# qzed/raft-meets-dicl

Hardware: AMD Instinct MI355X
Metric: frame-pairs/s @436x1024 RAFT 12 iters (1-8 GPU); corr MFMA% + lookup HBM% (higher is better)
Workload: dtype bf16; 1 GPU; RAFT all-pairs correlation + 4-level pyramid + 12 radius-4 lookups (BASELINE configs[1]); the whole network is the 'model_level' key; image=436x1024 padded 440x1024, feature_map=55x128, channels=256, batch_per_gpu=8, global_batch=8, precision=bf16, pyramid_storage=fp16, parallelism=batch-shard x1

## Files before the change

include/rmd.h:

```cpp
#ifndef RMD_H
#define RMD_H

#include <stddef.h>

#ifdef __cplusplus
extern "C" {
#endif

#define RMD_OK 0
#define RMD_ERR_ARG (-1)
#define RMD_ERR_SHAPE (-2)
#define RMD_ERR_LAUNCH (-3)

#define RMD_F32 0
#define RMD_F16 1
#define RMD_BF16 2
#define RMD_BF16X3 3
#define RMD_S24 4

#define RMD_MAX_LEVELS 4

#define RMD_LAYOUT_ROWS 0
#define RMD_LAYOUT_TILES 1

typedef struct rmd_pyramid_desc {
    int batch, height, width;
    int levels;
    int storage;
    int level_h[RMD_MAX_LEVELS], level_w[RMD_MAX_LEVELS];
    int tile_h[RMD_MAX_LEVELS], tile_w[RMD_MAX_LEVELS];
    int tiles_y[RMD_MAX_LEVELS], tiles_x[RMD_MAX_LEVELS];
    long long level_offset[RMD_MAX_LEVELS];
    long long total_elements;
    int layout;
    int query_slots;
} rmd_pyramid_desc;

int rmd_pyramid_describe(int batch, int height, int width, int levels, int storage,
                         rmd_pyramid_desc* desc);

int rmd_pyramid_describe_layout(int batch, int height, int width, int levels, int storage, int layout,
                                rmd_pyramid_desc* desc);

int rmd_pyramid_describe_for(int batch, int height, int width, int levels, int storage, int channels,
                             int compute, rmd_pyramid_desc* desc);

size_t rmd_corr_pyramid_workspace_bytes(const rmd_pyramid_desc* desc, int channels, int compute);

int rmd_corr_pyramid(const float* fmap1, const float* fmap2, int channels, float scale,
                     const rmd_pyramid_desc* desc, int compute, void* pyramid, void* workspace,
                     void* stream);

const char* rmd_corr_gemm_kernel(const rmd_pyramid_desc* desc, int channels, int compute);

int rmd_corr_prepare(const float* fmap1, const float* fmap2, int channels, float scale,
                     const rmd_pyramid_desc* desc, int compute, void* workspace, void* stream);
int rmd_corr_pyramid_prepared(int channels, float scale, const rmd_pyramid_desc* desc, int compute,
                              void* pyramid, void* workspace, void* stream);

int rmd_corr_lookup(const void* pyramid, const rmd_pyramid_desc* desc, const float* coords,
                    int radius, unsigned zero_level_mask, float* out, void* stream);

size_t rmd_corr_otf_workspace_bytes(int batch, int channels, int height, int width, int levels, int compute);
int rmd_corr_otf_prepare(const float* fmap1, const float* fmap2, int batch, int channels, int height, int width,
                         int levels, float scale, int compute, void* workspace, void* stream);
int rmd_corr_otf_lookup(const void* workspace, int batch, int channels, int height, int width, int levels,
                        int compute, const float* coords, int radius, unsigned zero_level_mask, float* out,
                        void* stream);

size_t rmd_corr_otf_record_bytes(int batch, int height, int width, int levels, int radius);
int rmd_corr_otf_record(const float* grad_out, const float* coords, int batch, int height, int width, int levels,
                        int radius, unsigned zero_level_mask, void* record, void* stream);
size_t rmd_corr_otf_backward_workspace_bytes(int batch, int channels, int height, int width, int levels, int compute);
int rmd_corr_otf_backward(const float* fmap1, const float* fmap2, const void* otf_workspace, int batch, int channels,
                          int height, int width, int levels, float scale, int compute, int radius, int nrecords,
                          const void* const* records, float* grad_fmap1, float* grad_fmap2, void* workspace,
                          void* stream);


long long rmd_corr_grad_targets(int height, int width, int levels);

int rmd_corr_lookup_backward(const float* grad_out, const rmd_pyramid_desc* desc, const float* coords,
                             int radius, unsigned zero_level_mask, float* grad_levels, void* stream);

int rmd_corr_grad_build(const float* const* grad_outs, const float* const* coords,
                        const unsigned* zero_level_masks, int nlookups, const rmd_pyramid_desc* desc, int radius,
                        int accumulate, float* grad_levels, void* stream);

int rmd_corr_grad_build_ex(const float* const* grad_outs, const float* const* coords,
                           const unsigned* zero_level_masks, int nlookups, const rmd_pyramid_desc* desc, int radius,
                           int accumulate, int bf16_out, void* grad_levels, void* stream);

int rmd_corr_pool_targets(const float* fmap2, int batch, int channels, int height, int width, int levels,
                          float scale, float* pooled, void* stream);

int rmd_corr_unpool_targets(const float* grad_pooled, int batch, int channels, int height, int width, int levels,
                            float scale, float* grad_fmap2, void* stream);

size_t rmd_corr_grad_gemm_workspace_bytes(int batch, int m, int k, int nc);
int rmd_corr_grad_gemm(const float* a, long long lda, const float* bm, long long ldb, int batch, int m, int k, int nc,
                       int layout, int compute, float* out, void* workspace, void* stream);

int rmd_corr_grad_gemm_bf16g(const float* a, long long lda, const void* bm, long long ldb, int batch, int m, int k,
                             int nc, int layout, float* out, void* workspace, void* stream);


int rmd_dicl_stack(const float* fmap1, const float* fmap2, const float* coords, int batch, int channels,
                   int height, int width, int level_height, int level_width, int radius, int level,
                   int norm_height, int norm_width, int extra_delta, float* out, void* stream);

int rmd_dicl_stack_backward(const float* grad_stack, const float* coords, int batch, int channels,
// ... 201 lines not shown
```

raft-meets-dicl_amd/csrc/corr_pyramid.h:

```cpp
#pragma once

#include "mfma_bf16.h"

namespace rmd {


constexpr int kKC = 64;
inline int padded_channels(int C) { return (C + kKC - 1) / kKC * kKC; }

__device__ __forceinline__ unsigned pack_half2(float a, float b) {
    const __half2 h = __floats2half2_rn(a, b);
    return *reinterpret_cast<const unsigned*>(&h);
}

__device__ __forceinline__ void swap32(unsigned& x, unsigned& y) {
    auto r = __builtin_amdgcn_permlane32_swap(x, y, false, false);
    x = r[0];
    y = r[1];
}

#define RMD_ACC(acc, row, cg, k) (acc[2 * ((row) >> 2) + (cg)][((row) & 3) * 4 + (k)])


namespace x3 {

bool eligible(const rmd_pyramid_desc& d, int channels);
size_t workspace_bytes(const rmd_pyramid_desc& d);
int prepare(const float* fmap1, const float* fmap2, int channels, float scale, const rmd_pyramid_desc& d,
            void* workspace, hipStream_t st);
int pyramid(const rmd_pyramid_desc& d, void* pyramid, void* workspace, hipStream_t st);

}

namespace w8 {

bool eligible(const rmd_pyramid_desc& d, int channels);
int prepare(const float* fmap1, const float* fmap2, int channels, float scale, const rmd_pyramid_desc& d,
            void* workspace, hipStream_t st);
int pyramid(const rmd_pyramid_desc& d, void* pyramid, void* workspace, hipStream_t st);

}

namespace stationary {

bool eligible(const rmd_pyramid_desc& d, int channels);
int pyramid(const rmd_pyramid_desc& d, void* pyramid, void* workspace, hipStream_t st);

}

namespace tiled {

int prepare(const float* fmap1, const float* fmap2, int channels, float scale, const rmd_pyramid_desc& d, int compute,
            void* workspace, hipStream_t st);
int pyramid(int channels, float scale, const rmd_pyramid_desc& d, int compute, void* pyramid, void* workspace,
            hipStream_t st);

}

}
```

raft-meets-dicl_amd/csrc/corr_pyramid.hip:

```cpp

#include "corr_pyramid.h"

namespace rmd {
namespace {

enum class Path { W8, STATIONARY, TILED, X3 };

Path gemm_path(const rmd_pyramid_desc& d, int C, int compute) {
    if (compute == RMD_BF16X3) return x3::eligible(d, C) ? Path::X3 : Path::TILED;
    if (compute == RMD_BF16) {
        if (w8::eligible(d, C)) return Path::W8;
        if (stationary::eligible(d, C)) return Path::STATIONARY;
    }
    return Path::TILED;
}

int path_layout(Path p) { return p == Path::W8 ? RMD_LAYOUT_TILES : RMD_LAYOUT_ROWS; }

int tiled_compute(int compute) { return compute == RMD_BF16X3 ? RMD_F32 : compute; }

int check_args(const rmd_pyramid_desc* d, int channels, int compute) {
    RMD_REQUIRE(d, RMD_ERR_ARG, "rmd_corr_pyramid: null desc");
    RMD_REQUIRE(channels > 0, RMD_ERR_SHAPE, "rmd_corr_pyramid: channels must be > 0");
    RMD_REQUIRE(d->levels >= 1 && d->levels <= RMD_MAX_LEVELS, RMD_ERR_SHAPE, "rmd_corr_pyramid: bad levels");
// ... 26 lines not shown
}

extern "C" size_t rmd_corr_pyramid_workspace_bytes(const rmd_pyramid_desc* d, int channels, int compute) {
    if (!d || channels <= 0) return 0;
    if (compute == RMD_BF16X3) {
        if (rmd::x3::eligible(*d, channels)) return rmd::x3::workspace_bytes(*d);
        compute = RMD_F32;
    }
    const size_t Cp = (size_t)rmd::padded_channels(channels);
    const size_t es = compute == RMD_F32 ? 4 : 2;
    const size_t N = (size_t)d->height * d->width;
    const size_t S = d->query_slots > 0 && (size_t)d->query_slots > N ? (size_t)d->query_slots : N;
    const size_t Npad = (S + 31) / 32 * 32;
    return (size_t)d->batch * (N + Npad) * Cp * es + 32 * 1024;
}

extern "C" const char* rmd_corr_gemm_kernel(const rmd_pyramid_desc* d, int channels, int compute) {
    if (!d || channels <= 0) return "invalid";
    switch (rmd::gemm_path(*d, channels, compute)) {
        case rmd::Path::W8: return "w8";
        case rmd::Path::STATIONARY: return "stationary";
        case rmd::Path::X3: return "x3";
        default: return "tiled";
    }
}

extern "C" int rmd_corr_prepare(const float* fmap1, const float* fmap2, int channels, float scale,
                                const rmd_pyramid_desc* d, int compute, void* workspace, void* stream) {
    RMD_REQUIRE(fmap1 && fmap2 && workspace, RMD_ERR_ARG, "rmd_corr_prepare: null pointer");
    int rc = rmd::check_args(d, channels, compute);
    if (rc) return rc;
    hipStream_t st = rmd::as_stream(stream);
    switch (rmd::gemm_path(*d, channels, compute)) {
        case rmd::Path::X3: return rmd::x3::prepare(fmap1, fmap2, channels, scale, *d, workspace, st);
        case rmd::Path::W8: return rmd::w8::prepare(fmap1, fmap2, channels, scale, *d, workspace, st);
        default: return rmd::tiled::prepare(fmap1, fmap2, channels, scale, *d, rmd::tiled_compute(compute), workspace, st);
    }
}

extern "C" int rmd_corr_pyramid_prepared(int channels, float scale, const rmd_pyramid_desc* d, int compute,
                                         void* pyramid, void* workspace, void* stream) {
    RMD_REQUIRE(pyramid && workspace, RMD_ERR_ARG, "rmd_corr_pyramid_prepared: null pointer");
    int rc = rmd::check_args(d, channels, compute);
    if (rc) return rc;
    hipStream_t st = rmd::as_stream(stream);
    switch (rmd::gemm_path(*d, channels, compute)) {
        case rmd::Path::X3: return rmd::x3::pyramid(*d, pyramid, workspace, st);
        case rmd::Path::W8: return rmd::w8::pyramid(*d, pyramid, workspace, st);
        case rmd::Path::STATIONARY: return rmd::stationary::pyramid(*d, pyramid, workspace, st);
        default: return rmd::tiled::pyramid(channels, scale, *d, rmd::tiled_compute(compute), pyramid, workspace, st);
    }
}

extern "C" int rmd_corr_pyramid(const float* fmap1, const float* fmap2, int channels, float scale,
                                const rmd_pyramid_desc* d, int compute, void* pyramid, void* workspace, void* stream) {
    int rc = rmd_corr_prepare(fmap1, fmap2, channels, scale, d, compute, workspace, stream);
    if (rc) return rc;
    return rmd_corr_pyramid_prepared(channels, scale, d, compute, pyramid, workspace, stream);
}
```

raft-meets-dicl_amd/csrc/corr_pyramid_w8.hip:

```cpp

#include "corr_pyramid.h"

namespace rmd {
namespace {

constexpr int kPrepPx = 128, kPrepStride = 256 * 2 + 16;

__global__ void __launch_bounds__(512)
prep_pair(const float* __restrict__ f1, const float* __restrict__ f2, __bf16* __restrict__ opA,
          __bf16* __restrict__ opB, int C, int H, int W, int S, int nqt, float scale) {
    extern __shared__ __attribute__((aligned(16))) unsigned char lds[];
    const int b = blockIdx.y, which = blockIdx.z;
    const int N = H * W;
    const float* f = which ? f1 : f2;
    const float s = which ? 1.0f : scale;
    const int t = threadIdx.x;
    const int p0 = blockIdx.x * kPrepPx;
    if (p0 >= (which ? S : N)) return;
#pragma unroll
    for (int it = 0; it < 2; ++it) {
        const int item = it * 512 + t;
        const int q = item & 31, cg = item >> 5;
        int y1, x1;
        if (which) {
            tiles_pixel(p0 + 4 * q, H, W, y1, x1);
        } else {
            y1 = 0;
            x1 = p0 + 4 * q;
        }
        const int lim = which ? W : N;
        const bool full = (which ? y1 < H : true) && x1 + 3 < lim && (lim & 3) == 0;
        const int yc = which ? min(y1, H - 1) : 0;
        const float* src = f + ((size_t)b * C) * N + (size_t)yc * (which ? W : 0);
        float v[8][4];
#pragma unroll
        for (int e = 0; e < 8; ++e) {
            const int c = cg * 8 + e;
            const float* row = src + (size_t)c * N;
            float4 x = make_float4(0.f, 0.f, 0.f, 0.f);
            if (c < C) {
                if (full) {
                    x = *reinterpret_cast<const float4*>(row + x1);
                } else {
                    x.x = row[min(x1 + 0, lim - 1)];
                    x.y = row[min(x1 + 1, lim - 1)];
                    x.z = row[min(x1 + 2, lim - 1)];
                    x.w = row[min(x1 + 3, lim - 1)];
                }
            }
            v[e][0] = x.x * s;
            v[e][1] = x.y * s;
            v[e][2] = x.z * s;
            v[e][3] = x.w * s;
        }
#pragma unroll
        for (int i = 0; i < 4; ++i) {
            bf16x8 o;
#pragma unroll
            for (int e = 0; e < 8; ++e) o[e] = (__bf16)v[e][i];
            *reinterpret_cast<bf16x8*>(lds + (size_t)(4 * q + i) * kPrepStride + cg * 16) = o;
        }
    }
    __syncthreads();
#pragma unroll
    for (int it = 0; it < 8; ++it) {
        const int k = it * 512 + t;
        int px, c0;
        if (which) {
            const int L = k & 63, st = (k >> 6) & 15;
            px = (k >> 10) * 32 + (L & 31);
            c0 = 16 * st + 8 * (L >> 5);
        } else {
            px = k >> 5;
            c0 = (k & 31) * 8;
        }
        const bf16x8 o = *reinterpret_cast<const bf16x8*>(lds + (size_t)px * kPrepStride + c0 * 2);
        if (which) {
            const int qt = blockIdx.x * 4 + (k >> 10);
            if (qt < nqt) *reinterpret_cast<bf16x8*>(opB + (((size_t)b * nqt + qt) * 1024 + (k & 1023)) * 8) = o;
        } else if (p0 + px < N) {
            *reinterpret_cast<bf16x8*>(opA + ((size_t)b * N + p0) * 256 + (size_t)k * 8) = o;
        }
    }
}


constexpr unsigned kBig = 0x40000000u;

constexpr int kStoreAux = 2;

struct Lvl {
    __amdgpu_buffer_rsrc_t rsrc;
    unsigned rs;
    unsigned cs;
    unsigned hd;
    int nq;
};

struct Ctx {
    Lvl l[4];
};

struct LaneOff {
    unsigned o0[2];
    unsigned o1;
    unsigned o2;
    unsigned o3;
};

__device__ __forceinline__ LaneOff lane_offsets(const Ctx& c, int q, int h) {
    LaneOff r;
    const unsigned uq = (unsigned)q;
#pragma unroll
    for (int tc = 0; tc < 2; ++tc)
        r.o0[tc] = 2 * tc + h < c.l[0].nq ? uq * 16u + (unsigned)(2 * tc + h) * c.l[0].cs : kBig;
    r.o1 = h < c.l[1].nq ? uq * 16u + (unsigned)h * c.l[1].cs : kBig;
    r.o2 = c.l[2].nq > 0 ? uq * 8u + (unsigned)h * c.l[2].rs : kBig;
    r.o3 = c.l[3].nq > 0 ? uq * 4u + (unsigned)h * (c.l[3].rs + c.l[3].hd) : kBig;
    return r;
}

struct EpiState {
    float s1[8][2][2];
    float s2[4][2];
};

#define V(row, cg, k) RMD_ACC(acc, row, cg, k)

template <int S>
__device__ __forceinline__ void epi_piece(const f32x16 (&acc)[8], const Ctx& c, const LaneOff& lo, EpiState& st) {
    constexpr int m = S >> 1, tc = S & 1;
    {
        const i32x4 d = {(int)pack_half2(V(2 * m, tc, 0), V(2 * m, tc, 1)),
                         (int)pack_half2(V(2 * m, tc, 2), V(2 * m, tc, 3)),
                         (int)pack_half2(V(2 * m + 1, tc, 0), V(2 * m + 1, tc, 1)),
                         (int)pack_half2(V(2 * m + 1, tc, 2), V(2 * m + 1, tc, 3))};
        __builtin_amdgcn_raw_buffer_store_b128(d, c.l[0].rsrc,
                                               (int)(lo.o0[tc] + (unsigned)m * c.l[0].rs + (m >= 4 ? c.l[0].hd : 0u)),
// ... 40 lines not shown
        swap32(x1, y1);
        const float inv = 1.0f / 64.0f;
        const unsigned v = pack_half2(inv * (__uint_as_float(x0) + __uint_as_float(y0)),
                                      inv * (__uint_as_float(x1) + __uint_as_float(y1)));
        __builtin_amdgcn_raw_buffer_store_b32((int)v, c.l[3].rsrc, (int)lo.o3, 0, kStoreAux);
    }
}
#undef V

constexpr unsigned kPadRow = 528;

__device__ __forceinline__ int pad_row(int y, int x) { return ((x >> 3) << 7) + (y << 3) + (x & 7); }

constexpr int kEpiStores = 24;
constexpr int kRing = 8;

template <int S>
__device__ __forceinline__ void read_a8(bf16x8 (&a)[8], const unsigned char* smem, unsigned b0, unsigned b1) {
#pragma unroll
    for (int ti = 0; ti < 8; ++ti)
        a[ti] = *reinterpret_cast<const bf16x8*>(smem + ((ti & 1) ? b1 : b0) + (unsigned)((ti >> 1) * 32 * kPadRow + 32 * S));
}

template <int S>
__device__ __forceinline__ void ksteps_ring(f32x16 (&acc)[8], bf16x8 (&acur)[8], bf16x8 (&anext)[8],
                                            bf16x8 (&ring)[kRing], const unsigned char* smem, unsigned b0,
                                            unsigned b1, const __bf16* cur, const __bf16* nxt) {
    if constexpr (S < 16) {
        if constexpr (S + 1 < 16) read_a8<S + 1>(anext, smem, b0, b1);
        {
            constexpr int T = S + kRing - 1;
            ring[T % kRing] = *reinterpret_cast<const bf16x8*>((T < 16 ? cur : nxt) + 512 * (T & 15));
        }
        const f32x16 zero = {};
#pragma unroll
        for (int ti = 0; ti < 8; ++ti)
            acc[ti] = __builtin_amdgcn_mfma_f32_32x32x16_bf16(acur[ti], ring[S % kRing], S == 0 ? zero : acc[ti], 0, 0, 0);
        if constexpr (S + 1 < 16) __builtin_amdgcn_sched_group_barrier(0x100, 8, 0);
        __builtin_amdgcn_sched_group_barrier(0x020, 1, 0);
        __builtin_amdgcn_sched_group_barrier(0x008, 8, 0);
        __builtin_amdgcn_sched_barrier(0);
        ksteps_ring<S + 1>(acc, anext, acur, ring, smem, b0, b1, cur, nxt);
    }
}

template <int S>
__device__ __forceinline__ void epilogue(const f32x16 (&acc)[8], const Ctx& c, const LaneOff& lo, EpiState& st) {
    if constexpr (S < 16) {
        epi_piece<S>(acc, c, lo, st);
        epilogue<S + 1>(acc, c, lo, st);
    }
}

struct Bal {
    int pair;
    int nwg;
};

__global__ void __launch_bounds__(512, 1)
corr_pyramid_w8(const __bf16* __restrict__ opA, const __bf16* __restrict__ opB, PyrGeom g, int qsplit,
                __half* __restrict__ pyr, Bal bal) {
    constexpr int Cp = 256, CPR = Cp / 8, WAVES = 8;
    extern __shared__ __attribute__((aligned(16))) unsigned char smem[];

    const int H = g.height, W = g.width, N = H * W;
    const int ncb = (W + 15) >> 4;
    const int nrb = (H + 15) >> 4;
    const int nqt = g.slots >> 5;
    const int nfull = bal.pair ? (nrb - 1) * ncb : nrb * ncb;
    const int nblk = nfull + (bal.pair ? ncb / 2 : 0);
    const int lid = xcd_block(blockIdx.x, bal.nwg);
    const int ib = lid % nblk;
    const int rest = lid / nblk;
    const int split = rest % qsplit;
    const int b = rest / qsplit;
    const bool paired = ib >= nfull;
    const int tb = paired ? (nrb - 1) * ncb + 2 * (ib - nfull) : ib;
    const int rb = tb / ncb, cb = tb - rb * ncb;
    const int ty0 = rb * 16, tx0 = cb * 16;
    const int tid = threadIdx.x, lane = tid & 63;
    const int w = __builtin_amdgcn_readfirstlane(tid >> 6);
    const int j = lane & 31, h = lane >> 5;

    const __bf16* gA = opA + (size_t)b * N * Cp;
    constexpr int kPieces = 256 * CPR / (64 * WAVES);
    uint4 av[kPieces];
#pragma unroll
    for (int i = 0; i < kPieces; ++i) {
        const int id = tid + i * 64 * WAVES;
        const int row = id / CPR, c = id - row * CPR;
        const bool second = paired && (row >> 4) >= 8;
        const int ty = ty0 + (row >> 4) - (second ? 8 : 0), tx = tx0 + (row & 15) + (second ? 16 : 0);
        av[i] = make_uint4(0, 0, 0, 0);
        if (ty < H && tx < W) av[i] = *reinterpret_cast<const uint4*>(gA + (size_t)(ty * W + tx) * Cp + c * 8);
    }
#pragma unroll
    for (int i = 0; i < kPieces; ++i) {
        const int id = tid + i * 64 * WAVES;
        const int row = id / CPR, c = id - row * CPR;
        *reinterpret_cast<uint4*>(smem + (size_t)pad_row(row >> 4, row & 15) * kPadRow + c * 16) = av[i];
    }
    __syncthreads();

    const unsigned pb0 = (unsigned)j * kPadRow + 16u * h, pb1 = pb0 + 128u * kPadRow;

    Ctx c;
    const unsigned S = (unsigned)g.slots;
#pragma unroll
    for (int l = 0; l < 4; ++l) {
        const int crows = l <= 1 ? 8 >> l : 4 >> (l - 2);
        const int cpb = l == 0 ? 4 : (l == 1 ? 2 : 1);
        const int cbytes = l <= 1 ? 16 : (l == 2 ? 8 : 4);
        const int cr0 = rb * crows, cc0 = cb * cpb;
        const bool lv = l < g.levels;
        const int rows = lv ? max(0, min(crows, g.ty[l] - cr0)) : 0;
        const unsigned cs = S * (unsigned)cbytes;
        const unsigned rs = lv ? (unsigned)g.tx[l] * cs : 0u;
        const size_t base = lv ? ((size_t)g.off[l] * 2 + (((size_t)b * g.ty[l] + cr0) * g.tx[l] + cc0) * (size_t)cs) : 0;
        const unsigned char* bp = reinterpret_cast<const unsigned char*>(pyr) + base;
        const unsigned lo32 = __builtin_amdgcn_readfirstlane((unsigned)(uintptr_t)bp);
        const unsigned hi32 = __builtin_amdgcn_readfirstlane((unsigned)((uintptr_t)bp >> 32));
        c.l[l].rsrc = __builtin_amdgcn_make_buffer_rsrc(reinterpret_cast<void*>(((uintptr_t)hi32 << 32) | lo32), (short)0,
                                                        (int)__builtin_amdgcn_readfirstlane((unsigned)rows * rs), 0x00020000);
        c.l[l].rs = __builtin_amdgcn_readfirstlane(rs);
        c.l[l].cs = __builtin_amdgcn_readfirstlane(cs);
        c.l[l].nq = __builtin_amdgcn_readfirstlane(lv ? max(0, min(cpb, g.tx[l] - cc0)) : 0);
        c.l[l].hd = paired ? __builtin_amdgcn_readfirstlane((unsigned)cpb * cs - (unsigned)(crows / 2) * rs) : 0u;
    }

    const __bf16* gB = opB + ((size_t)b * nqt * 1024 + lane) * 8;
    const int stride = WAVES * qsplit;
    const int f0 = split * WAVES;
    int qt = f0 + w;
    const int nmax = f0 < nqt ? (nqt - f0 + stride - 1) / stride : 0;
    const int nw = qt < nqt ? (nqt - qt + stride - 1) / stride : 0;
    const bool late = w >= 4;
    unsigned b0 = pb0, b1 = pb1;
    asm volatile("" : "+v"(b0), "+v"(b1));
    bf16x8 ring[kRing];
    if (nw > 0) {
#pragma unroll
        for (int s = 0; s < kRing - 1; ++s) ring[s] = *reinterpret_cast<const bf16x8*>(gB + (size_t)qt * 8192 + 512 * s);
    }
    vmcnt_pad_n<kEpiStores>(pyr);
    if (late) __builtin_amdgcn_s_barrier();
    for (int k = 0; k < nmax; ++k) {
        f32x16 acc[8];
        const int qn = qt + stride;
        if (k < nw) {
            bf16x8 a0[8], a1[8];
            read_a8<0>(a0, smem, b0, b1);
            ksteps_ring<0>(acc, a0, a1, ring, smem, b0, b1, gB + (size_t)qt * 8192,
                           gB + (size_t)min(qn, nqt - 1) * 8192);
            __builtin_amdgcn_s_barrier();
            const LaneOff lo = lane_offsets(c, qt * 32 + j, h);
            EpiState st;
            epilogue<0>(acc, c, lo, st);
            __builtin_amdgcn_s_barrier();
            qt = qn;
            continue;
        }
        __builtin_amdgcn_s_barrier();
        __builtin_amdgcn_s_barrier();
        qt = qn;
    }
    if (!late) __builtin_amdgcn_s_barrier();
}

long long tiles_slots(int H, int W) {
    return (long long)(H / 2) * ((W + 15) / 16) * 32 + ((H & 1) ? (long long)(W + 31) / 32 * 32 : 0);
}

Bal w8_balance(const rmd_pyramid_desc& d, int qs) {
    const int nrb = (d.height + 15) / 16, ncb = (d.width + 15) / 16;
    const int rows_last = d.height - 16 * (nrb - 1);
    if (qs == 1 && nrb >= 2 && rows_last <= 8 && d.width % 32 == 0) return {1, ((nrb - 1) * ncb + ncb / 2) * d.batch};
    return {0, nrb * ncb * d.batch * qs};
}

}

namespace w8 {

bool eligible(const rmd_pyramid_desc& d, int channels) {
    if (d.storage != RMD_F16 || padded_channels(channels) != 256) return false;
    const double slots = (double)tiles_slots(d.height, d.width);
    const double span0 = 16.0 * ((d.width + 7) / 8 * 8) * slots * 2;
    return span0 < (double)(1u << 30);
}

int prepare(const float* fmap1, const float* fmap2, int channels, float scale, const rmd_pyramid_desc& d,
            void* workspace, hipStream_t st) {
    const int N = d.height * d.width;
    __bf16* opA = reinterpret_cast<__bf16*>(workspace);
    __bf16* opB = opA + (size_t)d.batch * N * 256;
    const int S = d.query_slots;
    const int nqt = S / 32;
    const int lds = kPrepPx * kPrepStride;
    const int nx = ((N > S ? N : S) + kPrepPx - 1) / kPrepPx;
    (void)hipFuncSetAttribute(reinterpret_cast<const void*>(prep_pair), hipFuncAttributeMaxDynamicSharedMemorySize, lds);
    prep_pair<<<dim3(nx, d.batch, 2), 512, lds, st>>>(fmap1, fmap2, opA, opB, channels, d.height, d.width, S, nqt, scale);
    return check_launch("rmd_corr_prepare");
}

int pyramid(const rmd_pyramid_desc& d, void* pyramid, void* workspace, hipStream_t st) {
    const int N = d.height * d.width;
    __bf16* opA = reinterpret_cast<__bf16*>(workspace);
    __bf16* opB = opA + (size_t)d.batch * N * 256;
    const int nblk = ((d.height + 15) / 16) * ((d.width + 15) / 16);
    const int nqt = d.query_slots / 32;
    int qs = 1;
    while (nblk * d.batch * qs < 256 && qs * 32 <= nqt) qs *= 2;
    const int lds = 256 * (int)kPadRow;
    const Bal bal = w8_balance(d, qs);
    (void)hipFuncSetAttribute(reinterpret_cast<const void*>(corr_pyramid_w8), hipFuncAttributeMaxDynamicSharedMemorySize, lds);
    corr_pyramid_w8<<<bal.nwg, 512, lds, st>>>(opA, opB, make_geom(d), qs, reinterpret_cast<__half*>(pyramid), bal);
    return check_launch("rmd_corr_pyramid/gemm-w8");
}

}
}
```

raft-meets-dicl_amd/rmd/_lib.py:

```python

import ctypes
import hashlib
import os

import torch

RMD_OK = 0
RMD_F32, RMD_F16, RMD_BF16, RMD_BF16X3, RMD_S24 = 0, 1, 2, 3, 4
RMD_LAYOUT_ROWS, RMD_LAYOUT_TILES = 0, 1
RMD_NORM_NONE, RMD_NORM_INSTANCE = 0, 1
MAX_LEVELS = 4

_HERE = os.path.dirname(os.path.abspath(__file__))
LIB_PATH = os.environ.get("RMD_LIBRARY", os.path.join(_HERE, "librmd.so"))


class PyramidDesc(ctypes.Structure):

    _fields_ = [
        ("batch", ctypes.c_int), ("height", ctypes.c_int), ("width", ctypes.c_int),
        ("levels", ctypes.c_int), ("storage", ctypes.c_int),
        ("level_h", ctypes.c_int * MAX_LEVELS), ("level_w", ctypes.c_int * MAX_LEVELS),
        ("tile_h", ctypes.c_int * MAX_LEVELS), ("tile_w", ctypes.c_int * MAX_LEVELS),
        ("tiles_y", ctypes.c_int * MAX_LEVELS), ("tiles_x", ctypes.c_int * MAX_LEVELS),
        ("level_offset", ctypes.c_longlong * MAX_LEVELS),
        ("total_elements", ctypes.c_longlong),
        ("layout", ctypes.c_int), ("query_slots", ctypes.c_int),
    ]


LOSS_MAX_PREDICTIONS = 32
RMD_LOSS_L1, RMD_LOSS_L2, RMD_LOSS_ABSMEAN, RMD_LOSS_ROBUST = 1, 2, 3, 4


class LossPrediction(ctypes.Structure):

    _fields_ = [
        ("flow", ctypes.c_void_p), ("mask", ctypes.c_void_p), ("grad", ctypes.c_void_p),
        ("height", ctypes.c_int), ("width", ctypes.c_int), ("weight", ctypes.c_float),
    ]


METRICS_MAX_ESTIMATES, METRICS_MAX_DISTANCES, METRICS_SLOTS = 32, 8, 16


class RmdError(RuntimeError):
    pass


_lib = None

_P = ctypes.c_void_p
_I = ctypes.c_int
_U = ctypes.c_uint
_SIGS = {
    "rmd_pyramid_describe": (_I, [_I, _I, _I, _I, _I, ctypes.POINTER(PyramidDesc)]),
    "rmd_pyramid_describe_layout": (_I, [_I, _I, _I, _I, _I, _I, ctypes.POINTER(PyramidDesc)]),
    "rmd_pyramid_describe_for": (_I, [_I, _I, _I, _I, _I, _I, _I, ctypes.POINTER(PyramidDesc)]),
    "rmd_corr_pyramid_workspace_bytes": (ctypes.c_size_t, [ctypes.POINTER(PyramidDesc), _I, _I]),
    "rmd_corr_pyramid": (_I, [_P, _P, _I, ctypes.c_float, ctypes.POINTER(PyramidDesc), _I, _P, _P, _P]),
    "rmd_corr_lookup": (_I, [_P, ctypes.POINTER(PyramidDesc), _P, _I, _U, _P, _P]),
    "rmd_corr_gemm_kernel": (ctypes.c_char_p, [ctypes.POINTER(PyramidDesc), _I, _I]),
    "rmd_corr_prepare": (_I, [_P, _P, _I, ctypes.c_float, ctypes.POINTER(PyramidDesc), _I, _P, _P]),
    "rmd_corr_pyramid_prepared": (_I, [_I, ctypes.c_float, ctypes.POINTER(PyramidDesc), _I, _P, _P, _P]),
    "rmd_corr_otf_workspace_bytes": (ctypes.c_size_t, [_I] * 6),
    "rmd_corr_otf_prepare": (_I, [_P, _P] + [_I] * 5 + [ctypes.c_float, _I, _P, _P]),
    "rmd_corr_otf_lookup": (_I, [_P] + [_I] * 6 + [_P, _I, _U, _P, _P]),
    "rmd_corr_otf_record_bytes": (ctypes.c_size_t, [_I] * 5),
    "rmd_corr_otf_record": (_I, [_P, _P] + [_I] * 5 + [_U, _P, _P]),
    "rmd_corr_otf_backward_workspace_bytes": (ctypes.c_size_t, [_I] * 6),
    "rmd_corr_otf_backward": (_I, [_P, _P, _P] + [_I] * 5 + [ctypes.c_float, _I, _I, _I, ctypes.POINTER(_P), _P, _P,
                                                               _P, _P]),
    "rmd_corr_grad_targets": (ctypes.c_longlong, [_I, _I, _I]),
    "rmd_corr_lookup_backward": (_I, [_P, ctypes.POINTER(PyramidDesc), _P, _I, _U, _P, _P]),
    "rmd_corr_grad_build": (_I, [ctypes.POINTER(_P), ctypes.POINTER(_P), ctypes.POINTER(_U), _I,
                                 ctypes.POINTER(PyramidDesc), _I, _I, _P, _P]),
    "rmd_corr_grad_build_ex": (_I, [ctypes.POINTER(_P), ctypes.POINTER(_P), ctypes.POINTER(_U), _I,
                                    ctypes.POINTER(PyramidDesc), _I, _I, _I, _P, _P]),
    "rmd_corr_grad_gemm_bf16g": (_I, [_P, ctypes.c_longlong, _P, ctypes.c_longlong, _I, _I, _I, _I, _I, _P, _P, _P]),
    "rmd_corr_pool_targets": (_I, [_P, _I, _I, _I, _I, _I, ctypes.c_float, _P, _P]),
    "rmd_corr_unpool_targets": (_I, [_P, _I, _I, _I, _I, _I, ctypes.c_float, _P, _P]),
    "rmd_corr_grad_gemm_workspace_bytes": (ctypes.c_size_t, [_I, _I, _I, _I]),
    "rmd_corr_grad_gemm": (_I, [_P, ctypes.c_longlong, _P, ctypes.c_longlong, _I, _I, _I, _I, _I, _I, _P, _P, _P]),
    "rmd_dicl_stack": (_I, [_P, _P, _P] + [_I] * 11 + [_P, _P]),
    "rmd_dicl_stack_backward": (_I, [_P, _P] + [_I] * 11 + [_P, _P, _P]),
    "rmd_dicl_stack_kernel": (ctypes.c_char_p, [_I] * 12),
    "rmd_dicl_stack_kernel_list": (ctypes.c_char_p, [_I]),
    "rmd_dicl_stack_int_workspace_bytes": (ctypes.c_size_t, [_I, _I, _I]),
    "rmd_dicl_stack_int": (_I, [_P, _P] + [_I] * 6 + [_P, _P, _P]),
    "rmd_dicl_stack_int_backward": (_I, [_P, _P] + [_I] * 6 + [_P, _P, _P, _P]),
    "rmd_warp_backwards": (_I, [_P, _P, _I, _I, _I, _I, ctypes.c_float, _P, _P, _P]),
    "rmd_warp_backwards_backward": (_I, [_P, _P, _I, _I, _I, _I, ctypes.c_float, _P, _P]),
    "rmd_dicl_stack_int_warped_workspace_bytes": (ctypes.c_size_t, [_I, _I, _I, _I]),
    "rmd_dicl_stack_int_warped": (_I, [_P, _P, _P] + [_I] * 6 + [_P, _P, _P]),
    "rmd_dicl_stack_int_warped_backward": (_I, [_P, _P, _P] + [_I] * 6 + [_P, _P, _P, _P]),
    "rmd_dap": (_I, [_P, _P, _I, _I, _I, _I, _P, _P]),
    "rmd_dap_weight_grad_workspace_bytes": (ctypes.c_size_t, [_I, _I, _I]),
    "rmd_dap_weight_grad": (_I, [_P, _P, _I, _I, _I, _P, _P, _P]),
    "rmd_input_images": (_I, [_P, _I, _I, _I, _I, ctypes.c_float, ctypes.c_float, ctypes.c_float, ctypes.c_float,
                              _I, _I, _I, _I, _I, _P, _P]),
    "rmd_input_flow": (_I, [_P, _P, _I, _I, _I, _I, _I, _I, _I, ctypes.c_float, _P, _P, _P]),
    "rmd_up8": (_I, [_P, _P, _I, _I, _I, ctypes.c_float, _P, _P]),
    "rmd_up8_workspace_bytes": (ctypes.c_size_t, [_I, _I, _I]),
    "rmd_up8_backward": (_I, [_P, _P, _P, _I, _I, _I, ctypes.c_float, _P, _P, _P, _P]),
    "rmd_softargmax": (_I, [_P, _I, _I, _I, _I, _I, ctypes.c_float, _P, _P]),
    "rmd_softargmax_backward": (_I, [_P, _P, _I, _I, _I, _I, _I, ctypes.c_float, _P, _P]),
    "rmd_dicl_flow_head": (_I, [_P, _P, _I, _I, _I, _I, ctypes.c_float, _P, _P]),
    "rmd_dicl_flow_head_backward": (_I, [_P, _P, _I, _I, _I, _I, ctypes.c_float, _P, _P]),
    "rmd_dicl_match_1x1_supported": (_I, [_I] * 5),
    "rmd_dicl_match_1x1_workspace_bytes": (ctypes.c_size_t, [_I] * 5),
    "rmd_dicl_match_1x1": (_I, [_P, _P, _P] + [_I] * 5 + [_P] * 8 + [_I] * 4 + [_P, _P, _P]),
    "rmd_dicl_match_1x1_backward_supported": (_I, [_I] * 5),
    "rmd_dicl_match_1x1_backward_workspace_bytes": (ctypes.c_size_t, [_I] * 8),
    "rmd_dicl_match_1x1_backward": (_I, [_P] * 4 + [_I] * 5 + [_P] * 7 + [_I] * 4 + [_P] * 12),
    "rmd_sepconv_gru_supported": (_I, [_I] * 2),
    "rmd_sepconv_gru_workspace_bytes": (ctypes.c_size_t, [_I] * 5),
    "rmd_sepconv_gru": (_I, [_P] * 6 + [_I] * 6 + [_P]),
# ... 133 lines not shown
```

raft-meets-dicl_amd/rmd/library.py:

```python

import ctypes

import torch

from . import _lib

LIB = torch.library.Library("rmd", "DEF")

_OPS = {
    "corr_pyramid": ("model", "(Tensor fmap1, Tensor fmap2, int levels, int compute, int storage, float scale) "
                              "-> Tensor"),
    "corr_lookup": ("model", "(Tensor pyramid, Tensor coords, int levels, int radius, int level_mask) -> Tensor"),
    "corr_otf_prepare": ("model", "(Tensor fmap1, Tensor fmap2, int levels, int compute, float scale) -> Tensor"),
    "corr_otf_lookup": ("model", "(Tensor workspace, Tensor coords, int channels, int levels, int compute, int radius, "
                                 "int level_mask) -> Tensor"),
    "dicl_stack": ("model", "(Tensor fmap1, Tensor fmap2, Tensor coords, int radius, int level, int norm_h, "
                            "int norm_w, bool extra_delta) -> Tensor"),
    "dicl_stack_backward": ("model", "(Tensor grad, Tensor coords, int channels, int level_h, int level_w, int radius, "
                                     "int level, int norm_h, int norm_w, bool extra_delta) -> (Tensor, Tensor)"),
    "dicl_stack_int": ("model", "(Tensor fmap1, Tensor fmap2, int ru, int rv) -> Tensor"),
    "dicl_stack_int_backward": ("model", "(Tensor grad, Tensor fmap2, int ru, int rv) -> (Tensor, Tensor)"),
    "dicl_stack_int_warped": ("model", "(Tensor fmap1, Tensor fmap2, Tensor flow, int ru, int rv) -> Tensor"),
    "dicl_stack_int_warped_backward": ("model", "(Tensor grad, Tensor fmap2, Tensor flow, int ru, int rv) "
                                                "-> (Tensor, Tensor)"),
# ... 164 lines not shown
    elif pyramid.dim() == 2 and pyramid.shape[1] == TILES_ROW:
        return _lib.RMD_LAYOUT_TILES
    raise ValueError(f"corr_lookup: a pyramid is 1-D (row layout), (n, {TILES_ROW}) (tiles layout) or uint8 "
                     f"(n, {S24_BYTES}) (S24 storage), got {pyramid.dtype} {tuple(pyramid.shape)}")


def pyramid_storage(pyramid):
    if pyramid.dtype not in _STORAGE_CODE:
        raise ValueError(f"corr_lookup: pyramid dtype must be float32, float16 or uint8 (S24), got {pyramid.dtype}")
    return _STORAGE_CODE[pyramid.dtype]


def pyramid_elements(pyramid):
    return pyramid.shape[0] if pyramid.dtype == torch.uint8 else pyramid.numel()


def new_pyramid(like, d):
    if d.storage == _lib.RMD_S24:
        return like.new_empty((d.total_elements, S24_BYTES), dtype=torch.uint8)
    return pyramid_view(like.new_empty((d.total_elements,), dtype=_STORAGE[d.storage]), d.layout)


def pyramid_buffers(f1, levels, compute, storage):
    b, c, h, w = f1.shape
    d = describe_for(b, h, w, levels, storage, c, compute)
    ws = _lib.workspace("corr_pyramid", f1, ctypes.byref(d), c, compute)
    return d, new_pyramid(f1, d), ws


def s24_encode(x):
    u = _f32(x).reshape(-1).view(torch.int32)
    nan = (u & 0x7fffffff) > 0x7f800000
    r = torch.where(nan, u | 0x00400000, u + 0x80)
    return r.view(torch.uint8).view(-1, 4)[:, 1:4].contiguous()


def s24_decode(b):
    w = torch.zeros((b.shape[0], 4), dtype=torch.uint8, device=b.device)
    w[:, 1:4] = b
    return w.view(torch.float32).reshape(-1)



def _check_fmaps(f1, f2):
    if f1.shape != f2.shape or f1.dim() != 4:
        raise ValueError(f"fmap1/fmap2 must be equal (B,C,H,W) shapes, got {tuple(f1.shape)} / {tuple(f2.shape)}")


@_hip("corr_pyramid")
def _corr_pyramid(fmap1, fmap2, levels, compute, storage, scale):
    _check_fmaps(fmap1, fmap2)
    f1, f2 = _f32(fmap1), _f32(fmap2)
    d, data, ws = pyramid_buffers(f1, levels, compute, storage)
    _lib.launch("rmd_corr_pyramid", f1, f1, f2, f1.shape[1], float(scale), ctypes.byref(d), compute, data, ws)
    return data


@_fake("corr_pyramid")
def _(fmap1, fmap2, levels, compute, storage, scale):
    _check_fmaps(fmap1, fmap2)
    b, c, h, w = fmap1.shape
    if fmap1.device.type == "cpu":
        d = describe(b, h, w, levels, _lib.RMD_F32 if storage == _lib.RMD_S24 else storage)
    else:
        d = describe_for(b, h, w, levels, storage, c, compute)
    return new_pyramid(fmap1, d)


def _lookup_out(coords, levels, radius):
    b, _, h, w = coords.shape
    return _like(coords, (b, levels * (2 * radius + 1) ** 2, h, w))


@_hip("corr_lookup")
def _corr_lookup(pyramid, coords, levels, radius, level_mask):
    b, two, h, w = coords.shape
    if pyramid.dtype not in _STORAGE_CODE or not pyramid.is_contiguous():
        raise ValueError(f"corr_lookup: pyramid must be a contiguous float32/float16/uint8 (S24) tensor, got "
                         f"{pyramid.dtype} {tuple(pyramid.shape)}")
    d = describe(b, h, w, levels, pyramid_storage(pyramid), pyramid_layout(pyramid))
    if two != 2 or pyramid_elements(pyramid) != d.total_elements:
        raise ValueError(f"corr_lookup: coords {tuple(coords.shape)} do not match the pyramid ({pyramid.numel()} elements)")
    co = _f32(coords)
    out = _lookup_out(co, levels, radius)
    _lib.launch("rmd_corr_lookup", co, pyramid, ctypes.byref(d), co, radius, level_mask, out)
    return out


@_fake("corr_lookup")
def _(pyramid, coords, levels, radius, level_mask):
    pyramid_layout(pyramid)
    return _lookup_out(coords, levels, radius)


@_hip("corr_otf_prepare")
def _corr_otf_prepare(fmap1, fmap2, levels, compute, scale):
    _check_fmaps(fmap1, fmap2)
    f1, f2 = _f32(fmap1), _f32(fmap2)
    b, c, h, w = f1.shape
    ws = _lib.workspace("corr_otf", f1, b, c, h, w, levels, compute)
    if ws.numel() == 0:
        raise ValueError(f"otf: unsupported sizes {tuple(f1.shape)} with {levels} levels")
    _lib.launch("rmd_corr_otf_prepare", f1, f1, f2, b, c, h, w, levels, float(scale), compute, ws)
    return ws


@_fake("corr_otf_prepare")
# ... 1430 lines not shown
```

raft-meets-dicl_amd/rmd/ops.py:

```python

import ctypes

import torch

from . import _lib, config, library
from ._lib import RMD_BF16, RMD_BF16X3, RMD_F16, RMD_F32, RMD_S24
from .library import _f32

PRECISIONS = {
    "fp32": (RMD_BF16X3, RMD_S24),
    "fp32-f32": (RMD_BF16X3, RMD_F32),
    "fp32-s24": (RMD_BF16X3, RMD_S24),
    "fp32-exact": (RMD_F32, RMD_F32),
    "bf16": (RMD_BF16, RMD_F16),
    "bf16-f32": (RMD_BF16, RMD_F32),
    "fp32-f16": (RMD_F32, RMD_F16),
}


def set_default_precision(name):
    if name not in PRECISIONS:
        raise ValueError(f"unknown precision '{name}', expected one of {sorted(PRECISIONS)}")
    config.configure(precision=name)

# ... 21 lines not shown

class Pyramid:

    def __init__(self, data, desc, channels, scale):
        self.data = data
        self.desc = desc
        self.channels = channels
        self.scale = scale

    @property
    def levels(self):
        return self.desc.levels

    def level_shape(self, i):
        return self.desc.level_h[i], self.desc.level_w[i]

    def unpack(self, i):
        d = self.desc
        b, h, w = d.batch, d.height, d.width
        th, tw, ty, tx = d.tile_h[i], d.tile_w[i], d.tiles_y[i], d.tiles_x[i]
        hl, wl = d.level_h[i], d.level_w[i]
        s = d.query_slots
        off = d.level_offset[i]
        flat = library.s24_decode(self.data) if d.storage == RMD_S24 else self.data.reshape(-1)
        x = flat[off: off + b * ty * tx * s * th * tw].view(b, ty, tx, s, th, tw)
        x = x.permute(0, 3, 1, 4, 2, 5).reshape(b, s, ty * th, tx * tw)[..., :hl, :wl]
        if d.layout == _lib.RMD_LAYOUT_TILES:
            x = x.index_select(1, torch.as_tensor(tiles_slots(h, w), device=x.device))
        return x.float().reshape(b, h, w, 1, hl, wl)


def tiles_slots(h, w):
    y1, x1 = torch.meshgrid(torch.arange(h), torch.arange(w), indexing="ij")
    qx, hp = (w + 15) // 16, h // 2
    s = ((y1 // 2) * qx + x1 // 16) * 32 + ((x1 % 16) // 4) * 8 + (y1 % 2) * 4 + x1 % 4
    s = torch.where(y1 < 2 * hp, s, hp * qx * 32 + x1)
    return s.reshape(-1)


def corr_pyramid(fmap1, fmap2, levels=4, precision=None, events=None, scale=None):
    _same_device(fmap1, fmap2)
    if fmap1.shape != fmap2.shape or fmap1.dim() != 4:
        raise ValueError(f"fmap1/fmap2 must be equal (B,C,H,W) shapes, got {tuple(fmap1.shape)} / {tuple(fmap2.shape)}")
    compute, storage = PRECISIONS[precision or get_default_precision()]
    b, c, h, w = fmap1.shape
    scale = 1.0 / float(c) ** 0.5 if scale is None else float(scale)
    if events is None:
        data = torch.ops.rmd.corr_pyramid(fmap1, fmap2, levels, compute, storage, scale)
        d = library.describe(b, h, w, levels, library.pyramid_storage(data), library.pyramid_layout(data))
        return Pyramid(data, d, c, scale)
    _require_gpu(fmap1, fmap2)
    f1, f2 = _f32(fmap1), _f32(fmap2)
    d, data, ws = library.pyramid_buffers(f1, levels, compute, storage)
    with torch.cuda.device(f1.device):
        _lib.launch("rmd_corr_prepare", f1, f1, f2, c, scale, ctypes.byref(d), compute, ws)
        e0, e1 = torch.cuda.Event(enable_timing=True), torch.cuda.Event(enable_timing=True)
        e0.record()
        _lib.launch("rmd_corr_pyramid_prepared", f1, c, scale, ctypes.byref(d), compute, data, ws)
        e1.record()
        events.append((e0, e1))
    return Pyramid(data, d, c, scale)


def corr_lookup(pyr, coords, radius, mask_costs=()):
    _same_device(pyr.data, coords)
    d = pyr.desc
    if tuple(coords.shape) != (d.batch, 2, d.height, d.width):
        raise ValueError(f"coords must be (B,2,H,W)=({d.batch},2,{d.height},{d.width}), got {tuple(coords.shape)}")
    return torch.ops.rmd.corr_lookup(pyr.data, coords, d.levels, radius, _mask_bits(mask_costs, d.levels))



class OtfState:

    def __init__(self, ws, b, c, h, w, levels, compute):
        self.ws, self.b, self.c, self.h, self.w, self.levels, self.compute = ws, b, c, h, w, levels, compute


def otf_prepare(fmap1, fmap2, levels, precision=None, scale=1.0):
    _same_device(fmap1, fmap2)
    if fmap1.shape != fmap2.shape or fmap1.dim() != 4:
        raise ValueError(f"fmap1/fmap2 must be equal (B,C,H,W) shapes, got {tuple(fmap1.shape)} / {tuple(fmap2.shape)}")
    compute = PRECISIONS[precision or get_default_precision()][0]
    b, c, h, w = fmap1.shape
    ws = torch.ops.rmd.corr_otf_prepare(fmap1, fmap2, levels, compute, float(scale))
    return OtfState(ws, b, c, h, w, levels, compute)


def otf_lookup(st, coords, radius, mask_costs=()):
    _same_device(st.ws, coords)
    if tuple(coords.shape) != (st.b, 2, st.h, st.w):
        raise ValueError(f"coords must be (B,2,H,W)=({st.b},2,{st.h},{st.w}), got {tuple(coords.shape)}")
    return torch.ops.rmd.corr_otf_lookup(st.ws, coords, st.c, st.levels, st.compute, radius,
                                         _mask_bits(mask_costs, st.levels))



class _OtfState:
    def __init__(self, otf, f1, f2, scale):
        self.otf = otf
        self.f1 = f1
        self.f2 = f2
        self.scale = scale
        self.records = []
        self.radius = None


class _OtfPrepareFn(torch.autograd.Function):

    @staticmethod
    def forward(ctx, fmap1, fmap2, state):
# ... 545 lines not shown
```

Before: 15010 frame-pairs/s.

## Fuse fmap2 fp32-to-bf16 staging into the w8 correlation GEMM

```diff
diff --git a/include/rmd.h b/include/rmd.h
--- a/include/rmd.h
+++ b/include/rmd.h
@@ -57,6 +57,15 @@
                      const rmd_pyramid_desc* desc, int compute, void* workspace, void* stream);
 int rmd_corr_pyramid_prepared(int channels, float scale, const rmd_pyramid_desc* desc, int compute,
                               void* pyramid, void* workspace, void* stream);
+
+int rmd_corr_pyramid_fused(const float* fmap1, const float* fmap2, int channels, float scale,
+                           const rmd_pyramid_desc* desc, int compute, void* pyramid, void* workspace,
+                           void* stream);
+
+int rmd_corr_prepare_queries(const float* fmap1, int channels, const rmd_pyramid_desc* desc, int compute,
+                             void* workspace, void* stream);
+int rmd_corr_pyramid_staged(const float* fmap2, int channels, float scale, const rmd_pyramid_desc* desc,
+                            int compute, void* pyramid, void* workspace, void* stream);
 
 int rmd_corr_lookup(const void* pyramid, const rmd_pyramid_desc* desc, const float* coords,
                     int radius, unsigned zero_level_mask, float* out, void* stream);
diff --git a/raft-meets-dicl_amd/csrc/corr_pyramid.h b/raft-meets-dicl_amd/csrc/corr_pyramid.h
--- a/raft-meets-dicl_amd/csrc/corr_pyramid.h
+++ b/raft-meets-dicl_amd/csrc/corr_pyramid.h
@@ -38,6 +38,9 @@
 int prepare(const float* fmap1, const float* fmap2, int channels, float scale, const rmd_pyramid_desc& d,
             void* workspace, hipStream_t st);
 int pyramid(const rmd_pyramid_desc& d, void* pyramid, void* workspace, hipStream_t st);
+int prepare_queries(const float* fmap1, int channels, const rmd_pyramid_desc& d, void* workspace, hipStream_t st);
+int pyramid_staged(const float* fmap2, int channels, float scale, const rmd_pyramid_desc& d, void* pyramid,
+                   void* workspace, hipStream_t st);
 
 }
 
diff --git a/raft-meets-dicl_amd/csrc/corr_pyramid.hip b/raft-meets-dicl_amd/csrc/corr_pyramid.hip
--- a/raft-meets-dicl_amd/csrc/corr_pyramid.hip
+++ b/raft-meets-dicl_amd/csrc/corr_pyramid.hip
@@ -102,6 +102,39 @@
     }
 }
 
+extern "C" int rmd_corr_prepare_queries(const float* fmap1, int channels, const rmd_pyramid_desc* d, int compute,
+                                        void* workspace, void* stream) {
+    RMD_REQUIRE(fmap1 && workspace, RMD_ERR_ARG, "rmd_corr_prepare_queries: null pointer");
+    int rc = rmd::check_args(d, channels, compute);
+    if (rc) return rc;
+    RMD_REQUIRE(rmd::gemm_path(*d, channels, compute) == rmd::Path::W8, RMD_ERR_ARG,
+                "rmd_corr_prepare_queries: the w8 GEMM only (see rmd_corr_gemm_kernel)");
+    return rmd::w8::prepare_queries(fmap1, channels, *d, workspace, rmd::as_stream(stream));
+}
+
+extern "C" int rmd_corr_pyramid_staged(const float* fmap2, int channels, float scale, const rmd_pyramid_desc* d,
+                                       int compute, void* pyramid, void* workspace, void* stream) {
+    RMD_REQUIRE(fmap2 && pyramid && workspace, RMD_ERR_ARG, "rmd_corr_pyramid_staged: null pointer");
+    int rc = rmd::check_args(d, channels, compute);
+    if (rc) return rc;
+    RMD_REQUIRE(rmd::gemm_path(*d, channels, compute) == rmd::Path::W8, RMD_ERR_ARG,
+                "rmd_corr_pyramid_staged: the w8 GEMM only (see rmd_corr_gemm_kernel)");
+    return rmd::w8::pyramid_staged(fmap2, channels, scale, *d, pyramid, workspace, rmd::as_stream(stream));
+}
+
+extern "C" int rmd_corr_pyramid_fused(const float* fmap1, const float* fmap2, int channels, float scale,
+                                      const rmd_pyramid_desc* d, int compute, void* pyramid, void* workspace,
+                                      void* stream) {
+    RMD_REQUIRE(fmap1 && fmap2 && pyramid && workspace, RMD_ERR_ARG, "rmd_corr_pyramid_fused: null pointer");
+    int rc = rmd::check_args(d, channels, compute);
+    if (rc) return rc;
+    if (rmd::gemm_path(*d, channels, compute) != rmd::Path::W8)
+        return rmd_corr_pyramid(fmap1, fmap2, channels, scale, d, compute, pyramid, workspace, stream);
+    rc = rmd::w8::prepare_queries(fmap1, channels, *d, workspace, rmd::as_stream(stream));
+    if (rc) return rc;
+    return rmd::w8::pyramid_staged(fmap2, channels, scale, *d, pyramid, workspace, rmd::as_stream(stream));
+}
+
 extern "C" int rmd_corr_pyramid(const float* fmap1, const float* fmap2, int channels, float scale,
                                 const rmd_pyramid_desc* d, int compute, void* pyramid, void* workspace, void* stream) {
     int rc = rmd_corr_prepare(fmap1, fmap2, channels, scale, d, compute, workspace, stream);
diff --git a/raft-meets-dicl_amd/csrc/corr_pyramid_w8.hip b/raft-meets-dicl_amd/csrc/corr_pyramid_w8.hip
--- a/raft-meets-dicl_amd/csrc/corr_pyramid_w8.hip
+++ b/raft-meets-dicl_amd/csrc/corr_pyramid_w8.hip
@@ -6,11 +6,10 @@
 
 constexpr int kPrepPx = 128, kPrepStride = 256 * 2 + 16;
 
-__global__ void __launch_bounds__(512)
-prep_pair(const float* __restrict__ f1, const float* __restrict__ f2, __bf16* __restrict__ opA,
-          __bf16* __restrict__ opB, int C, int H, int W, int S, int nqt, float scale) {
+__device__ __forceinline__ void prep_tile(const int which, const float* f1, const float* f2, __bf16* opA, __bf16* opB,
+                                          int C, int H, int W, int S, int nqt, float scale) {
     extern __shared__ __attribute__((aligned(16))) unsigned char lds[];
-    const int b = blockIdx.y, which = blockIdx.z;
+    const int b = blockIdx.y;
     const int N = H * W;
     const float* f = which ? f1 : f2;
     const float s = which ? 1.0f : scale;
@@ -84,6 +83,17 @@
     }
 }
 
+__global__ void __launch_bounds__(512)
+prep_pair(const float* __restrict__ f1, const float* __restrict__ f2, __bf16* __restrict__ opA,
+          __bf16* __restrict__ opB, int C, int H, int W, int S, int nqt, float scale) {
+    prep_tile(blockIdx.z, f1, f2, opA, opB, C, H, W, S, nqt, scale);
+}
+
+__global__ void __launch_bounds__(512)
+prep_queries(const float* __restrict__ f1, __bf16* __restrict__ opB, int C, int H, int W, int S, int nqt) {
+    prep_tile(1, f1, nullptr, nullptr, opB, C, H, W, S, nqt, 1.0f);
+}
+
 
 constexpr unsigned kBig = 0x40000000u;
 
@@ -230,14 +240,70 @@
     }
 }
 
+struct StageItem {
+    int xq, cg, y;
+    int ty, tx;
+};
+
+__device__ __forceinline__ StageItem stage_item(int id, int ty0, int tx0, bool paired) {
+    StageItem t;
+    t.xq = id & 3, t.cg = (id >> 2) & 31, t.y = id >> 7;
+    const bool second = paired && t.y >= 8;
+    t.ty = ty0 + t.y - (second ? 8 : 0), t.tx = tx0 + 4 * t.xq + (second ? 16 : 0);
+    return t;
+}
+
+__device__ __forceinline__ void stage_write_px(unsigned char* smem, const StageItem& t, int i, const float (&p)[8], int C,
+                                               int H, int W, float scale) {
+    bf16x8 o;
+#pragma unroll
+    for (int e = 0; e < 8; ++e) o[e] = (__bf16)(t.ty < H && t.tx + i < W ? (t.cg * 8 + e < C ? p[e] : 0.0f) * scale : 0.0f);
+    *reinterpret_cast<bf16x8*>(smem + (size_t)pad_row(t.y, 4 * t.xq + i) * kPadRow + t.cg * 16) = o;
+}
+
+__device__ __forceinline__ void stage_a_f32(unsigned char* smem, const float* __restrict__ f2, int C, int H, int W,
+                                            float scale, int ty0, int tx0, bool paired, int tid) {
+    constexpr int kItems = 4;
+    const int N = H * W;
+    if ((W & 3) == 0 && (reinterpret_cast<uintptr_t>(f2) & 15) == 0 && N < (1 << 22)) {
+#pragma unroll 1
+        for (int it = 0; it < kItems; ++it) {
+            const StageItem t = stage_item(it * 512 + tid, ty0, tx0, paired);
+            const unsigned pix = (unsigned)(min(t.ty, H - 1) * W + min(t.tx, W - 4));
+            float4 x[8];
+#pragma unroll
+            for (int e = 0; e < 8; ++e) {
+                const unsigned c = (unsigned)min(t.cg * 8 + e, C - 1);
+                x[e] = *reinterpret_cast<const float4*>(reinterpret_cast<const unsigned char*>(f2) +
+                                                        (size_t)((c * (unsigned)N + pix) * 4u));
+            }
+            stage_write_px(smem, t, 0, {x[0].x, x[1].x, x[2].x, x[3].x, x[4].x, x[5].x, x[6].x, x[7].x}, C, H, W, scale);
+            stage_write_px(smem, t, 1, {x[0].y, x[1].y, x[2].y, x[3].y, x[4].y, x[5].y, x[6].y, x[7].y}, C, H, W, scale);
+            stage_write_px(smem, t, 2, {x[0].z, x[1].z, x[2].z, x[3].z, x[4].z, x[5].z, x[6].z, x[7].z}, C, H, W, scale);
+            stage_write_px(smem, t, 3, {x[0].w, x[1].w, x[2].w, x[3].w, x[4].w, x[5].w, x[6].w, x[7].w}, C, H, W, scale);
+        }
+        return;
+    }
+#pragma unroll 1
+    for (int k = 0; k < 4 * kItems; ++k) {
+        const StageItem t = stage_item((k >> 2) * 512 + tid, ty0, tx0, paired);
+        const int i = k & 3;
+        const float* px = f2 + (size_t)min(t.ty, H - 1) * W + min(t.tx + i, W - 1);
+        float p[8];
+#pragma unroll
+        for (int e = 0; e < 8; ++e) p[e] = px[(size_t)min(t.cg * 8 + e, C - 1) * N];
+        stage_write_px(smem, t, i, p, C, H, W, scale);
+    }
+}
+
 struct Bal {
     int pair;
     int nwg;
 };
 
-__global__ void __launch_bounds__(512, 1)
-corr_pyramid_w8(const __bf16* __restrict__ opA, const __bf16* __restrict__ opB, PyrGeom g, int qsplit,
-                __half* __restrict__ pyr, Bal bal) {
+template <bool kF32>
+__device__ __forceinline__ void w8_body(const void* srcA, int C, float scale, const __bf16* opB, const PyrGeom& g,
+                                        int qsplit, __half* pyr, const Bal& bal) {
     constexpr int Cp = 256, CPR = Cp / 8, WAVES = 8;
     extern __shared__ __attribute__((aligned(16))) unsigned char smem[];
 
@@ -260,23 +326,27 @@
     const int w = __builtin_amdgcn_readfirstlane(tid >> 6);
     const int j = lane & 31, h = lane >> 5;
 
-    const __bf16* gA = opA + (size_t)b * N * Cp;
-    constexpr int kPieces = 256 * CPR / (64 * WAVES);
-    uint4 av[kPieces];
-#pragma unroll
-    for (int i = 0; i < kPieces; ++i) {
-        const int id = tid + i * 64 * WAVES;
-        const int row = id / CPR, c = id - row * CPR;
-        const bool second = paired && (row >> 4) >= 8;
-        const int ty = ty0 + (row >> 4) - (second ? 8 : 0), tx = tx0 + (row & 15) + (second ? 16 : 0);
-        av[i] = make_uint4(0, 0, 0, 0);
-        if (ty < H && tx < W) av[i] = *reinterpret_cast<const uint4*>(gA + (size_t)(ty * W + tx) * Cp + c * 8);
-    }
-#pragma unroll
-    for (int i = 0; i < kPieces; ++i) {
-        const int id = tid + i * 64 * WAVES;
-        const int row = id / CPR, c = id - row * CPR;
-        *reinterpret_cast<uint4*>(smem + (size_t)pad_row(row >> 4, row & 15) * kPadRow + c * 16) = av[i];
+    if constexpr (kF32) {
+        stage_a_f32(smem, static_cast<const float*>(srcA) + (size_t)b * C * N, C, H, W, scale, ty0, tx0, paired, tid);
+    } else {
+        const __bf16* gA = static_cast<const __bf16*>(srcA) + (size_t)b * N * Cp;
+        constexpr int kPieces = 256 * CPR / (64 * WAVES);
+        uint4 av[kPieces];
+#pragma unroll
+        for (int i = 0; i < kPieces; ++i) {
+            const int id = tid + i * 64 * WAVES;
+            const int row = id / CPR, c = id - row * CPR;
+            const bool second = paired && (row >> 4) >= 8;
+            const int ty = ty0 + (row >> 4) - (second ? 8 : 0), tx = tx0 + (row & 15) + (second ? 16 : 0);
+            av[i] = make_uint4(0, 0, 0, 0);
+            if (ty < H && tx < W) av[i] = *reinterpret_cast<const uint4*>(gA + (size_t)(ty * W + tx) * Cp + c * 8);
+        }
+#pragma unroll
+        for (int i = 0; i < kPieces; ++i) {
+            const int id = tid + i * 64 * WAVES;
+            const int row = id / CPR, c = id - row * CPR;
+            *reinterpret_cast<uint4*>(smem + (size_t)pad_row(row >> 4, row & 15) * kPadRow + c * 16) = av[i];
+        }
     }
     __syncthreads();
 
@@ -345,6 +415,18 @@
     if (!late) __builtin_amdgcn_s_barrier();
 }
 
+__global__ void __launch_bounds__(512, 1)
+corr_pyramid_w8(const __bf16* __restrict__ opA, const __bf16* __restrict__ opB, PyrGeom g, int qsplit,
+                __half* __restrict__ pyr, Bal bal) {
+    w8_body<false>(opA, 0, 0.0f, opB, g, qsplit, pyr, bal);
+}
+
+__global__ void __launch_bounds__(512, 1)
+corr_pyramid_w8_f32(const float* __restrict__ f2, const __bf16* __restrict__ opB, PyrGeom g, int qsplit,
+                    __half* __restrict__ pyr, Bal bal, int C, float scale) {
+    w8_body<true>(f2, C, scale, opB, g, qsplit, pyr, bal);
+}
+
 long long tiles_slots(int H, int W) {
     return (long long)(H / 2) * ((W + 15) / 16) * 32 + ((H & 1) ? (long long)(W + 31) / 32 * 32 : 0);
 }
@@ -381,7 +463,21 @@
     return check_launch("rmd_corr_prepare");
 }
 
-int pyramid(const rmd_pyramid_desc& d, void* pyramid, void* workspace, hipStream_t st) {
+int prepare_queries(const float* fmap1, int channels, const rmd_pyramid_desc& d, void* workspace, hipStream_t st) {
+    const int N = d.height * d.width;
+    __bf16* opB = reinterpret_cast<__bf16*>(workspace) + (size_t)d.batch * N * 256;
+    const int S = d.query_slots;
+    const int lds = kPrepPx * kPrepStride;
+    (void)hipFuncSetAttribute(reinterpret_cast<const void*>(prep_queries), hipFuncAttributeMaxDynamicSharedMemorySize, lds);
+    prep_queries<<<dim3((S + kPrepPx - 1) / kPrepPx, d.batch), 512, lds, st>>>(fmap1, opB, channels, d.height, d.width, S,
+                                                                                S / 32);
+    return check_launch("rmd_corr_prepare_queries");
+}
+
+namespace {
+
+int launch_gemm(const float* fmap2, int channels, float scale, const rmd_pyramid_desc& d, void* pyramid, void* workspace,
+                hipStream_t st) {
     const int N = d.height * d.width;
     __bf16* opA = reinterpret_cast<__bf16*>(workspace);
     __bf16* opB = opA + (size_t)d.batch * N * 256;
@@ -391,10 +487,28 @@
     while (nblk * d.batch * qs < 256 && qs * 32 <= nqt) qs *= 2;
     const int lds = 256 * (int)kPadRow;
     const Bal bal = w8_balance(d, qs);
+    if (fmap2) {
+        (void)hipFuncSetAttribute(reinterpret_cast<const void*>(corr_pyramid_w8_f32),
+                                  hipFuncAttributeMaxDynamicSharedMemorySize, lds);
+        corr_pyramid_w8_f32<<<bal.nwg, 512, lds, st>>>(fmap2, opB, make_geom(d), qs, reinterpret_cast<__half*>(pyramid), bal,
+                                                       channels, scale);
+        return check_launch("rmd_corr_pyramid/gemm-w8-f32");
+    }
     (void)hipFuncSetAttribute(reinterpret_cast<const void*>(corr_pyramid_w8), hipFuncAttributeMaxDynamicSharedMemorySize, lds);
     corr_pyramid_w8<<<bal.nwg, 512, lds, st>>>(opA, opB, make_geom(d), qs, reinterpret_cast<__half*>(pyramid), bal);
     return check_launch("rmd_corr_pyramid/gemm-w8");
 }
 
 }
-}
+
+int pyramid(const rmd_pyramid_desc& d, void* pyramid, void* workspace, hipStream_t st) {
+    return launch_gemm(nullptr, 0, 0.0f, d, pyramid, workspace, st);
+}
+
+int pyramid_staged(const float* fmap2, int channels, float scale, const rmd_pyramid_desc& d, void* pyramid,
+                   void* workspace, hipStream_t st) {
+    return launch_gemm(fmap2, channels, scale, d, pyramid, workspace, st);
+}
+
+}
+}
diff --git a/raft-meets-dicl_amd/rmd/_lib.py b/raft-meets-dicl_amd/rmd/_lib.py
--- a/raft-meets-dicl_amd/rmd/_lib.py
+++ b/raft-meets-dicl_amd/rmd/_lib.py
@@ -63,6 +63,9 @@
     "rmd_corr_gemm_kernel": (ctypes.c_char_p, [ctypes.POINTER(PyramidDesc), _I, _I]),
     "rmd_corr_prepare": (_I, [_P, _P, _I, ctypes.c_float, ctypes.POINTER(PyramidDesc), _I, _P, _P]),
     "rmd_corr_pyramid_prepared": (_I, [_I, ctypes.c_float, ctypes.POINTER(PyramidDesc), _I, _P, _P, _P]),
+    "rmd_corr_pyramid_fused": (_I, [_P, _P, _I, ctypes.c_float, ctypes.POINTER(PyramidDesc), _I, _P, _P, _P]),
+    "rmd_corr_prepare_queries": (_I, [_P, _I, ctypes.POINTER(PyramidDesc), _I, _P, _P]),
+    "rmd_corr_pyramid_staged": (_I, [_P, _I, ctypes.c_float, ctypes.POINTER(PyramidDesc), _I, _P, _P, _P]),
     "rmd_corr_otf_workspace_bytes": (ctypes.c_size_t, [_I] * 6),
     "rmd_corr_otf_prepare": (_I, [_P, _P] + [_I] * 5 + [ctypes.c_float, _I, _P, _P]),
     "rmd_corr_otf_lookup": (_I, [_P] + [_I] * 6 + [_P, _I, _U, _P, _P]),
diff --git a/raft-meets-dicl_amd/rmd/library.py b/raft-meets-dicl_amd/rmd/library.py
--- a/raft-meets-dicl_amd/rmd/library.py
+++ b/raft-meets-dicl_amd/rmd/library.py
@@ -240,7 +240,7 @@
     _check_fmaps(fmap1, fmap2)
     f1, f2 = _f32(fmap1), _f32(fmap2)
     d, data, ws = pyramid_buffers(f1, levels, compute, storage)
-    _lib.launch("rmd_corr_pyramid", f1, f1, f2, f1.shape[1], float(scale), ctypes.byref(d), compute, data, ws)
+    _lib.launch("rmd_corr_pyramid_fused", f1, f1, f2, f1.shape[1], float(scale), ctypes.byref(d), compute, data, ws)
     return data
 
 
diff --git a/raft-meets-dicl_amd/rmd/ops.py b/raft-meets-dicl_amd/rmd/ops.py
--- a/raft-meets-dicl_amd/rmd/ops.py
+++ b/raft-meets-dicl_amd/rmd/ops.py
@@ -97,11 +97,18 @@
     _require_gpu(fmap1, fmap2)
     f1, f2 = _f32(fmap1), _f32(fmap2)
     d, data, ws = library.pyramid_buffers(f1, levels, compute, storage)
+    staged = _lib.lib().rmd_corr_gemm_kernel(ctypes.byref(d), c, compute) == b"w8"
     with torch.cuda.device(f1.device):
-        _lib.launch("rmd_corr_prepare", f1, f1, f2, c, scale, ctypes.byref(d), compute, ws)
+        if staged:
+            _lib.launch("rmd_corr_prepare_queries", f1, f1, c, ctypes.byref(d), compute, ws)
+        else:
+            _lib.launch("rmd_corr_prepare", f1, f1, f2, c, scale, ctypes.byref(d), compute, ws)
         e0, e1 = torch.cuda.Event(enable_timing=True), torch.cuda.Event(enable_timing=True)
         e0.record()
-        _lib.launch("rmd_corr_pyramid_prepared", f1, c, scale, ctypes.byref(d), compute, data, ws)
+        if staged:
+            _lib.launch("rmd_corr_pyramid_staged", f1, f2, c, scale, ctypes.byref(d), compute, data, ws)
+        else:
+            _lib.launch("rmd_corr_pyramid_prepared", f1, c, scale, ctypes.byref(d), compute, data, ws)
         e1.record()
         events.append((e0, e1))
     return Pyramid(data, d, c, scale)
```

Result: faster. 15330 frame-pairs/s (median of 6 runs) (+2.1%).
